# artiom-matvei/RLAO

Hardware: AMD Instinct MI355X
Metric: AO env-steps/sec (batched loops) (higher is better)
Workload: dtype f32; 1 GPU; 8m / 20x20 Shack-Hartmann, 256 batched envs per GPU, integrator closed loop (BASELINE.json configs[1]); envs_per_gpu=256, envs_total=256, resolution=120, n_valid_act=357, n_signal=632, layers=1, controller=leaky integrator, gain 0.5, noise=photon, parallelism=env-shards x1, all-gather of episode returns

## Files before the change

rlao_amd/csrc/common.hpp:

```cpp
#pragma once
#include <hip/hip_runtime.h>
#include <stdint.h>
#include <stddef.h>

#include <string>
#include <vector>

#include "aoenv.h"

namespace ao {

constexpr int kWave = 64;
constexpr int kMaxLayer = 8;
constexpr int kMtN = 624;
constexpr int kMaxSplits = 16;
constexpr int kMaxModes = 512;

int fail(const char* fmt, ...);
#define AO_HIP(call)                                                                          \
    do {                                                                                      \
        hipError_t e_ = (call);                                                               \
        if (e_ != hipSuccess)                                                                 \
            return ::ao::fail("%s:%d: %s -> %s", __FILE__, __LINE__, #call, hipGetErrorString(e_)); \
    } while (0)
// ... 29 lines not shown
    w[1] = 0.5 * (3 * x * x * x - 5 * x * x + 2);
    w[2] = 0.5 * (-3 * x * x * x + 4 * x * x + x);
    w[3] = 0.5 * (x * x * x - x * x);
}

__host__ __device__ inline bool clock_subpixel(const double ratio[2], double buff[2], int* bx, int* by) {
#pragma clang fp contract(off)
    for (int d = 0; d < 2; ++d) buff[d] += fmod(fabs(ratio[d]), 1.0) * clock_sgn(ratio[d]);
    *bx = fabs(buff[0]) < 1 ? 0 : (int)clock_sgn(buff[0]);
    *by = fabs(buff[1]) < 1 ? 0 : (int)clock_sgn(buff[1]);
    for (int d = 0; d < 2; ++d) buff[d] = fmod(fabs(buff[d]), 1.0) * clock_sgn(buff[d]);
    return *bx != 0 || *by != 0;
}

__host__ __device__ inline void taps_from_buff(const double buff[2], LayerTaps& t) {
#pragma clang fp contract(off)
    const double fy = -buff[1], fx = -buff[0];
    const double ky = floor(fy), kx = floor(fx);
    t.dy = (int)ky;
    t.dx = (int)kx;
    catmull_rom(fy - ky, t.wy);
    catmull_rom(fx - kx, t.wx);
}

struct PhaseArgs {
    const void* screen[kMaxLayer];
    const void* minmax[kMaxLayer];
    LayerTaps taps[kMaxLayer];
    int n_layer;
    int S;
    int foot;
    int S_l[kMaxLayer];
    int foot_l[kMaxLayer];
    int update_atm;
    int store_atm;
    int store_phase;
    int minmax_dirty[kMaxLayer];
    const LayerTaps* env_taps;
    int n_env;
};

__device__ inline const LayerTaps& layer_taps(const PhaseArgs& pa, int l, int e) {
    return pa.env_taps ? pa.env_taps[(size_t)l * pa.n_env + e] : pa.taps[l];
}

}

namespace ao {

struct Env;

template <typename T>
int launch_ring_prepare(const T* map, T* zx, const int* inner_idx, const uint32_t* mt_state, const int* mt_pos,
                        uint32_t* mt_state_out, int* mt_pos_out, const int* env_idx, int n, int S, int n_inner, int n_outer, int K,
                        int sx, int sy, int oy, int ox, const double* xi_scale, hipStream_t st);
template <typename T>
int launch_mt_normal(uint32_t* mt_state, int* mt_pos, T* zx, int n_env, int K, int n_inner, int n_outer,
                     const double* xi_scale, hipStream_t st);
template <typename T>
int launch_scatter_minmax(T* new_map, const T* X, const int* outer_idx, T* minmax, const int* env_idx, int n, int n_env, int S,
                          int n_outer, int splits, int oy, int ox, int with_minmax, hipStream_t st, const LayerTaps* env_taps = nullptr);
template <typename T>
int launch_ring_prepare_env(const T* map, T* zx, const int* inner_idx, uint32_t* mt_state, int* mt_pos, const EnvClock* clk_in,
                            EnvClock* clk_out, LayerTaps* taps, double weight, int n_env, int S, int n_inner, int n_outer, int K,
                            const double* xi_scale, hipStream_t st);
template <typename T>
int launch_minmax(const T* maps, T* minmax, int n_env, int S, hipStream_t st);
int launch_mt_seed(const uint32_t* seeds, int stride, const int* env_idx, uint32_t* mt_state, int* mt_pos, int n, hipStream_t st);
template <typename T>
int launch_reset_env_rows(const int* env_idx, int n_idx, T* coefs, T* dm_prev, int n_valid_act, EnvClock* clk, LayerTaps* taps,
                          int n_layer, int n_env, hipStream_t st);
int gemm_splits(int M, int N, int K);
struct MtAhead {
    const uint32_t* mt_in;
    const int* pos_in;
    uint32_t* mt_out;
    int* pos_out;
    float* zx_out;
    int K, n_inner, n_outer, n_env;
    const double* xi_scale;
};
int launch_ring_gemm_draw_ahead(const float* X, const float* W, float* Cpart, int M, int N, int K, int splits, const MtAhead& m,
                                hipStream_t st);
int launch_sum_slabs(float* x, size_t n, int slabs, hipStream_t st);
int launch_gemm_nt_mfma(const float* X, const float* W, float* Cpart, int M, int N, int K, int ldx, int ldw, int splits,
                        hipStream_t st, int xsplits = 1, size_t xslab = 0);
template <typename T>
int launch_gemm_nt(const T* X, const T* W, T* C, int M, int N, int K, int ldx, int ldw, int ldc, hipStream_t st);

__host__ __device__ inline size_t ga_index(int x, int k, int ga_stride) {
    const int q = k & 3, s = k >> 2;
    return ((((size_t)(x >> 4) * (ga_stride >> 2) + (s >> 2)) * 4 + q) * 16 + (x & 15)) * 4 + (s & 3);
}
template <typename T>
struct PhaseBuffers {
    T* opd_atm;
    const T* coefs;
    const T* coefs_img;
    const T* dm_opd;
    const T* gx;
    const T* gy;
    const T* gxt;
    const float* gxa;
    const float* gya;
    int ga_stride;
    const float* s1a;
    const int* act_idx;
    const uint8_t* pupil;
    T* phase;
    double* part;
    T* wfs_max;
};
int phase_tiles(int R, int n_act, size_t esz);
template <typename T>
int launch_coefs_image(const T* coefs, const int* act_idx, T* img, int n_env, int n_act, int n_valid_act, hipStream_t st);
int launch_dm_rows(const float* coefs, const int* act_idx, const float* gya, float* s1a, int n_env, int R, int n_act, int n_valid_act,
                   int ga_stride, hipStream_t st);
template <typename T>
struct KArgs {
    PhaseArgs pa;
    PhaseBuffers<T> pb;
    int R, n_act, n_valid_act, tx, rp;
    T atm_scale;
    T src_scale;
};
template <typename T>
KArgs<T> make_phase_kargs(const PhaseArgs& pa, const PhaseBuffers<T>& pb, int R, int n_act, int n_valid_act,
                          double atm_wavelength, double src_wavelength);
template <typename T>
int launch_phase(const PhaseArgs& pa, const PhaseBuffers<T>& pb, int n_env, int R, int n_act, int n_valid_act,
                 double atm_wavelength, double src_wavelength, bool use_mfma, int force_path, hipStream_t st);

template <typename T>
struct ShConst {
    const T* amp;
    const int* subap_idx;
    const uint8_t* valid2d;
    const T* ref;
    const T* tw;
    const T* ph;
    T units;
    T threshold;
    int fast_trig;
};
template <typename T>
int launch_sh_spots(const T* phase, const ShConst<T>& sc, T* frame, T* wfs_max, int n_env, int R, int n_subap,
                    int n_valid, hipStream_t st);
template <typename T>
int launch_sh_centroid(const T* frame, const T* wfs_max, const ShConst<T>& sc, T* signal, int n_env, int R,
                       int n_subap, int n_valid, int max_group, hipStream_t st);

template <typename T>
struct FinishArgs {
    const T* v;
    int splits;
    const int* act_idx;
    const T* action;
    T* coefs;
    T* dm_prev;
    T* obs;
    T* reward;
    T* ret;
    T* strehl;
    T* scal;
    T* total;
    T* residual;
// ... 120 lines not shown
```

rlao_amd/csrc/env.hip:

```cpp
#include <algorithm>
#include <cmath>
#include <cstdarg>
#include <cstdio>
#include <cstring>
#include <initializer_list>
#include <new>
#include <utility>

#include "common.hpp"
#include "detector.hpp"
#include "sh_device.hpp"

namespace ao {

static thread_local std::string g_err;

int fail(const char* fmt, ...) {
    char buf[1024];
    va_list ap;
    va_start(ap, fmt);
    vsnprintf(buf, sizeof(buf), fmt, ap);
    va_end(ap);
    g_err = buf;
    return 1;
// ... 202 lines not shown
    sc.fast_trig = (env->use_fast_trig && sizeof(T) == 4) ? 1 : 0;
    return sc;
}

template <typename T>
int gemm_dispatch(AoEnv* env, const T* X, const T* W, T* C, int M, int N, int K, int* splits, hipStream_t st);
template <>
int gemm_dispatch<float>(AoEnv* env, const float* X, const float* W, float* C, int M, int N, int K, int* splits,
                         hipStream_t st) {
    if (!env->use_mfma) { *splits = 1; return launch_gemm_nt<float>(X, W, C, M, N, K, K, K, N, st); }
    *splits = gemm_splits(M, N, K);
    return launch_gemm_nt_mfma(X, W, C, M, N, K, K, K, *splits, st);
}
template <>
int gemm_dispatch<double>(AoEnv*, const double* X, const double* W, double* C, int M, int N, int K, int* splits,
                          hipStream_t st) {
    *splits = 1;
    return launch_gemm_nt<double>(X, W, C, M, N, K, K, K, N, st);
}

void forget_lookahead(Layer& y) { y.ahead.valid = false; y.gather_next = false; }

void drop_ring(Layer& y) { y.ring_pending = 0; }

void move_origin(Layer& y, int sx, int sy) {
    y.org[0] = ((y.org[0] - sy) % y.S + y.S) % y.S;
    y.org[1] = ((y.org[1] - sx) % y.S + y.S) % y.S;
}

void defer_ring(AoEnv* env, int l, const void* zx, int splits) {
    env->last_zx = zx;
    env->last_zx_layer = l;
    env->layer[l].ring_pending = splits;
    env->layer[l].ring_src = env->xbuf_ptr(l);
}

void take_rings(AoEnv* env, StepArgs& a) {
    for (int l = 0; l < env->L; ++l) {
        Layer& y = env->layer[l];
        a.ring_x[l] = y.ring_pending ? static_cast<const float*>(y.ring_src) : nullptr;
        a.ring_splits[l] = y.ring_pending;
        const bool g = y.gather_next && y.ring_pending && y.ahead.valid;
        a.next_zx[l] = g ? static_cast<float*>(env->zx_pipe_ptr(y.ahead.buf, l)) : nullptr;
        a.next_sx[l] = y.ahead.sx;
        a.next_sy[l] = y.ahead.sy;
        if (y.gather_next && !g) y.ahead.valid = false;
        y.gather_next = false;
    }
}

void rings_written(AoEnv* env) {
    for (int l = 0; l < env->L; ++l) { env->layer[l].ring_pending = 0; env->layer[l].minmax_dirty = false; }
}

template <typename T>
int scatter_ring(AoEnv* env, int l, const LayerTaps* et, bool with_minmax, hipStream_t st) {
    Layer& y = env->layer[l];
    AO_PROF(env, SCATTER, st);
    AO_TRY(launch_scatter_minmax<T>(env->as<T>(env->screen_ptr(l)), static_cast<const T*>(y.ring_src), y.outer_idx,
                                    env->as<T>(env->minmax_ptr(l)), nullptr, env->E, env->E, y.S, y.nout, y.ring_pending, y.org[0],
                                    y.org[1], with_minmax ? 1 : 0, st, et));
    y.ring_pending = 0;
    return 0;
}

template <typename T>
int flush_ring(AoEnv* env, int l, hipStream_t st) {
    Layer& y = env->layer[l];
    if (!y.ring_pending) return 0;
    if (y.gather_next) forget_lookahead(y);
    const LayerTaps* et = env->per_env_wind ? env->env_taps + (size_t)l * env->E : nullptr;
    return scatter_ring<T>(env, l, et, et != nullptr, st);
}
template <typename T>
int flush_rings(AoEnv* env, hipStream_t st) {
    for (int l = 0; l < env->L; ++l) AO_TRY(flush_ring<T>(env, l, st));
    return 0;
}

template <typename T>
int ring_gemm(AoEnv* env, int l, const T* zx, int* splits, hipStream_t st) {
    const Layer& y = env->layer[l];
    AO_PROF(env, GEMM_RING, st);
    return gemm_dispatch<T>(env, zx, env->as<T>(y.ab), env->as<T>(env->xbuf_ptr(l)), env->E, y.nout, y.K, splits, st);
}

template <typename T>
int extrude(AoEnv* env, int l, int sx, int sy, bool lean, hipStream_t st, bool defer = false) {
    Layer& y = env->layer[l];
    forget_lookahead(y);
    AO_TRY(flush_ring<T>(env, l, st));
    T* zx = env->as<T>(env->zx);
    {
        AO_PROF(env, SHIFT_GATHER, st);
        AO_TRY(launch_ring_prepare<T>(env->as<T>(env->screen_ptr(l)), zx, y.inner_idx, y.mt_cur, y.pos_cur, y.mt_cur, y.pos_cur, nullptr,
                                      env->E, y.S, y.nin, y.nout, y.K, sx, sy, y.org[0], y.org[1], env->sigma(), st));
    }
    int splits = 1;
    AO_TRY(ring_gemm<T>(env, l, zx, &splits, st));
    move_origin(y, sx, sy);
    defer_ring(env, l, zx, splits);
    if (!(defer && lean)) AO_TRY(scatter_ring<T>(env, l, nullptr, !lean, st));
    y.minmax_dirty = lean;
    return 0;
}

template <typename T>
int first_ring(AoEnv* env, int l, const int* d_idx, int n, hipStream_t st) {
    Layer& y = env->layer[l];
    T* zx = env->as<T>(env->zx);
    T* map = env->as<T>(env->screen_ptr(l));
    {
        AO_PROF(env, SHIFT_GATHER, st);
        AO_TRY(launch_ring_prepare<T>(map, zx, y.inner_idx, y.mt_cur, y.pos_cur, y.mt_cur, y.pos_cur, d_idx, n, y.S, y.nin, y.nout, y.K, 0, 0,
                                      0, 0, env->sigma(), st));
    }
    int splits = 1;
    AO_TRY(ring_gemm<T>(env, l, zx, &splits, st));
    env->last_zx = zx;
    env->last_zx_layer = l;
    {
        AO_PROF(env, SCATTER, st);
        AO_TRY(launch_scatter_minmax<T>(map, env->as<T>(env->xbuf_ptr(l)), y.outer_idx, env->as<T>(env->minmax_ptr(l)), d_idx, n, env->E,
                                        y.S, y.nout, splits, 0, 0, 1, st));
    }
    if (!d_idx) y.minmax_dirty = false;
    return 0;
}

template <typename T>
int refresh_minmax(AoEnv* env, hipStream_t st) {
    AO_TRY(flush_rings<T>(env, st));
    for (int l = 0; l < env->L; ++l)
        if (env->layer[l].minmax_dirty) {
            AO_TRY(launch_minmax<T>(env->as<T>(env->screen_ptr(l)), env->as<T>(env->minmax_ptr(l)), env->E, env->layer[l].S, st));
            env->layer[l].minmax_dirty = false;
        }
    return 0;
}

bool next_crossing(const LayerClock& k0, int* sx, int* sy) {
    if ((int)std::fabs(k0.ratio[0]) > 0 || (int)std::fabs(k0.ratio[1]) > 0) return false;
    if (k0.ratio[0] == 0 && k0.ratio[1] == 0) return false;
    double b[2] = {k0.buff[0], k0.buff[1]};
    for (int it = 0; it < 1000000; ++it) {
        for (int d = 0; d < 2; ++d) b[d] += std::fmod(std::fabs(k0.ratio[d]), 1.0) * sgn(k0.ratio[d]);
        if (std::fabs(b[0]) >= 1 || std::fabs(b[1]) >= 1) {
            *sx = std::fabs(b[0]) < 1 ? 0 : (int)sgn(b[0]);
            *sy = std::fabs(b[1]) < 1 ? 0 : (int)sgn(b[1]);
            return true;
        }
        for (int d = 0; d < 2; ++d) b[d] = std::fmod(std::fabs(b[d]), 1.0) * sgn(b[d]);
    }
    return false;
}

int extrude_pipelined(AoEnv* env, int l, int sx, int sy, hipStream_t st) {
    Layer& y = env->layer[l];
    const int cur = y.ahead.buf;
    float* op = static_cast<float*>(env->zx_pipe_ptr(cur, l));
    if (y.ahead.valid && y.ahead.sx == sx && y.ahead.sy == sy) {
        std::swap(y.mt_cur, y.mt_alt);
        std::swap(y.pos_cur, y.pos_alt);
    } else {
        AO_PROF(env, SHIFT_GATHER, st);
        AO_TRY(launch_ring_prepare<float>(env->as<float>(env->screen_ptr(l)), op, y.inner_idx, y.mt_cur, y.pos_cur, y.mt_cur, y.pos_cur,
                                          nullptr, env->E, y.S, y.nin, y.nout, y.K, sx, sy, y.org[0], y.org[1], env->sigma(), st));
    }
    forget_lookahead(y);
    const int splits = gemm_splits(env->E, y.nout, y.K);
    MtAhead m{y.mt_cur, y.pos_cur, y.mt_alt, y.pos_alt, static_cast<float*>(env->zx_pipe_ptr(1 - cur, l)), y.K, y.nin, y.nout, env->E,
              env->sigma()};
    {
        AO_PROF(env, GEMM_RING, st);
        AO_TRY(launch_ring_gemm_draw_ahead(op, env->as<float>(y.ab), static_cast<float*>(env->xbuf_ptr(l)), env->E, y.nout, y.K, splits, m,
                                           st));
    }
    move_origin(y, sx, sy);
    defer_ring(env, l, op, splits);
    y.minmax_dirty = true;
    int nsx = 0, nsy = 0;
    if (next_crossing(y.clk, &nsx, &nsy)) {
        y.ahead = RingAhead{true, nsx, nsy, 1 - cur};
        y.gather_next = true;
    }
    return 0;
}

template <typename T>
int advance_atmosphere_env(AoEnv* env, bool lean, hipStream_t st) {
    for (int l = 0; l < env->L; ++l) {
        AO_TRY(flush_ring<T>(env, l, st));
        const Layer& y = env->layer[l];
        T* zx = env->as<T>(env->zx);
        const size_t row = (size_t)l * env->E;
        {
            AO_PROF(env, SHIFT_GATHER, st);
            AO_TRY(launch_ring_prepare_env<T>(env->as<T>(env->screen_ptr(l)), zx, y.inner_idx, y.mt_cur, y.pos_cur,
                                              env->env_clk[env->clk_cur] + row, env->env_clk[1 - env->clk_cur] + row, env->env_taps + row,
                                              y.weight, env->E, y.S, y.nin, y.nout, y.K, env->sigma(), st));
        }
        int splits = 1;
        AO_TRY(ring_gemm<T>(env, l, zx, &splits, st));
        defer_ring(env, l, zx, splits);
        if (!(lean && env->defer_ring)) AO_TRY(flush_ring<T>(env, l, st));
    }
    env->clk_cur = 1 - env->clk_cur;
    return 0;
}

template <typename T>
int advance_atmosphere(AoEnv* env, bool lean, hipStream_t st) {
    if (env->per_env_wind) return advance_atmosphere_env<T>(env, lean, st);
    for (int l = 0; l < env->L; ++l) {
        LayerClock& k = env->layer[l].clk;
        if (k.ratio[0] == 0 && k.ratio[1] == 0) continue;
        const int ns[2] = {(int)std::fabs(k.ratio[0]), (int)std::fabs(k.ratio[1])};
        const int mn = ns[0] < ns[1] ? ns[0] : ns[1], mx = ns[0] > ns[1] ? ns[0] : ns[1];
        const int s0 = (int)sgn(k.ratio[0]), s1 = (int)sgn(k.ratio[1]);
        for (int i = 0; i < mn; ++i) AO_TRY(extrude<T>(env, l, s0, s1, lean, st));
        for (int j = 0; j < mx - mn; ++j)
            AO_TRY(extrude<T>(env, l, ns[0] == mn ? 0 : s0, ns[1] == mn ? 0 : s1, lean, st));
        int b0, b1;
        if (clock_subpixel(k.ratio, k.buff, &b0, &b1)) {
            if (lean && env->defer_ring && env->use_lookahead && env->zx_pipe && !env->layer[l].ring_pending) {
                AO_TRY(extrude_pipelined(env, l, b0, b1, st));
            } else {
                AO_TRY(extrude<T>(env, l, b0, b1, lean, st, lean && env->defer_ring));
            }
        }
    }
    return 0;
}

template <typename T>
void fill_phase_args(AoEnv* env, PhaseArgs& pa, PhaseBuffers<T>& pb, int update_atm, int store_atm, int store_phase);

template <typename T>
int run_phase(AoEnv* env, int update_atm, int store_atm, hipStream_t st, int store_phase = 1) {
    AO_TRY(refresh_minmax<T>(env, st));
    if (env->use_coefs_img && env->c.dm_separable) {
        if constexpr (std::is_same<T, float>::value) {
            if (env->dm_rows)
                AO_TRY(launch_dm_rows(env->as<float>(env->coefs), env->act_idx, env->gya, env->dm_rows, env->E, env->R, env->nAct, env->A,
                                      env->ga_stride, st));
        }
        if (env->coefs_img)
            AO_TRY(launch_coefs_image<T>(env->as<T>(env->coefs), env->act_idx, env->as<T>(env->coefs_img), env->E, env->nAct, env->A, st));
    }
    PhaseArgs pa;
    PhaseBuffers<T> pb;
    fill_phase_args<T>(env, pa, pb, update_atm, store_atm, store_phase);
    AO_PROF(env, PHASE, st);
    return launch_phase<T>(pa, pb, env->E, env->R, env->nAct, env->A, env->c.atm_wavelength, env->c.src_wavelength,
                           env->use_mfma, env->force_path, st);
}

template <typename T>
int apply_detector(AoEnv* env, bool sh, hipStream_t st) {
    if (!env->det.active) return 0;
    env->det.frame_counter += 1;
    AO_PROF(env, DETECTOR, st);
// ... 1551 lines not shown
```

rlao_amd/csrc/gemm_kernels.hip:

```cpp
#include "common.hpp"
#include "ring_device.hpp"

namespace ao {

template <typename T>
__global__ void __launch_bounds__(256) k_gemm_nt(const T* __restrict__ X, const T* __restrict__ W, T* __restrict__ C,
                                                 int M, int N, int K, int ldx, int ldw, int ldc) {
    constexpr int BM = 64, BN = 64, BK = 16;
    __shared__ T xs[BK][BM + 1];
    __shared__ T ws[BK][BN + 1];
    const int m0 = blockIdx.y * BM, n0 = blockIdx.x * BN;
    const int tx = threadIdx.x % 16, ty = threadIdx.x / 16;
    T acc[4][4];
#pragma unroll
    for (int i = 0; i < 4; ++i)
#pragma unroll
        for (int j = 0; j < 4; ++j) acc[i][j] = (T)0;

    for (int k0 = 0; k0 < K; k0 += BK) {
        for (int q = threadIdx.x; q < BM * BK; q += 256) {
            const int r = q / BK, kk = q % BK;
            const int gm = m0 + r, gn = n0 + r, gk = k0 + kk;
            xs[kk][r] = (gm < M && gk < K) ? X[(size_t)gm * ldx + gk] : (T)0;
            ws[kk][r] = (gn < N && gk < K) ? W[(size_t)gn * ldw + gk] : (T)0;
// ... 63 lines not shown
                if (gm < M) {
                    xv[pass] = *reinterpret_cast<const float4*>(X + (size_t)gm * ldx + gk);
                    for (int z = 1; z < xsplits; ++z) {
                        const float4 t = *reinterpret_cast<const float4*>(X + (size_t)z * xslab + (size_t)gm * ldx + gk);
                        xv[pass].x += t.x; xv[pass].y += t.y; xv[pass].z += t.z; xv[pass].w += t.w;
                    }
                }
                if (gn < N) wv[pass] = *reinterpret_cast<const float4*>(W + (size_t)gn * ldw + gk);
            } else {
                float* xp = reinterpret_cast<float*>(&xv[pass]);
                float* wp = reinterpret_cast<float*>(&wv[pass]);
                for (int d = 0; d < 4; ++d) {
                    if (gk + d < kend) {
                        if (gm < M) {
                            xp[d] = X[(size_t)gm * ldx + gk + d];
                            for (int z = 1; z < xsplits; ++z) xp[d] += X[(size_t)z * xslab + (size_t)gm * ldx + gk + d];
                        }
                        if (gn < N) wp[d] = W[(size_t)gn * ldw + gk + d];
                    }
                }
            }
        }
    };
    if (kbeg < kend) fetch(kbeg);
    for (int k0 = kbeg; k0 < kend; k0 += BK) {
#pragma unroll
        for (int pass = 0; pass < 2; ++pass) {
            const int r = (threadIdx.x >> 3) + pass * 32, kq = (threadIdx.x & 7) * 4;
            float* xd = xs + r * LDT + kq;
            float* wd = ws + r * LDT + kq;
            xd[0] = xv[pass].x; xd[1] = xv[pass].y; xd[2] = xv[pass].z; xd[3] = xv[pass].w;
            wd[0] = wv[pass].x; wd[1] = wv[pass].y; wd[2] = wv[pass].z; wd[3] = wv[pass].w;
        }
        __syncthreads();
        if (k0 + BK < kend) fetch(k0 + BK);
        const float* xa = xs + (wm + lr) * LDT + lh;
        const float* wb = ws + (wn + lr) * LDT + lh;
#pragma unroll
        for (int kk = 0; kk < BK / 2; ++kk)
            acc = __builtin_amdgcn_mfma_f32_32x32x2f32(xa[2 * kk], wb[2 * kk], acc, 0, 0, 0);
        __syncthreads();
    }
    float* C = Cpart + (size_t)bz * M * N;
    const int gn = n0 + wn + lr;
    if (gn < N) {
#pragma unroll
        for (int rg = 0; rg < 16; ++rg) {
            const int gm = m0 + wm + (rg & 3) + 8 * (rg >> 2) + 4 * lh;
            if (gm < M) C[(size_t)gm * N + gn] = acc[rg];
        }
    }
}

__global__ void __launch_bounds__(256) k_gemm_nt_mfma(const float* __restrict__ X, const float* __restrict__ W,
                                                      float* __restrict__ Cpart, int M, int N, int K, int ldx,
                                                      int ldw, int kslice, int xsplits, size_t xslab) {
    gemm_nt_mfma_tile(X, W, Cpart, M, N, K, ldx, ldw, kslice, xsplits, xslab, (int)blockIdx.z);
}

__global__ void __launch_bounds__(256) k_ring_gemm_draw_ahead(const float* __restrict__ X, const float* __restrict__ W,
                                                              float* __restrict__ Cpart, int M, int N, int K, int ldx, int ldw,
                                                              int kslice, int splits, const MtAhead m) {
    const int draw_slices = (int)gridDim.z - splits;
    if ((int)blockIdx.z >= draw_slices) {
        gemm_nt_mfma_tile(X, W, Cpart, M, N, K, ldx, ldw, kslice, 1, 0, (int)blockIdx.z - draw_slices);
        return;
    }
    const int e = ((int)blockIdx.z * (int)gridDim.y + (int)blockIdx.y) * (int)gridDim.x + (int)blockIdx.x;
    if (e < m.n_env) mt_normal_body<float>(m.mt_in, m.pos_in, m.mt_out, m.pos_out, m.zx_out, m.K, m.n_inner, m.n_outer, e,
                                           m.xi_scale);
}

int launch_ring_gemm_draw_ahead(const float* X, const float* W, float* Cpart, int M, int N, int K, int splits, const MtAhead& m,
                                hipStream_t st) {
    if (m.n_outer % 2) return fail("mt_normal: n_outer=%d must be even", m.n_outer);
    const int kslice = cdiv(cdiv(K, splits), 32) * 32;
    const int gx = cdiv(N, 64), gy = cdiv(M, 64);
    dim3 grid(gx, gy, splits + cdiv(m.n_env, gx * gy));
    hipLaunchKernelGGL(k_ring_gemm_draw_ahead, grid, dim3(256), 0, st, X, W, Cpart, M, N, K, K, K, kslice, splits, m);
    AO_HIP(hipGetLastError());
    return 0;
}

int gemm_splits(int M, int N, int K) {
    const int tiles = cdiv(M, 64) * cdiv(N, 64);
    if (K > 2048) {
        int best = 1;
        double best_cost = 1e300;
        for (int s = 1; s <= kMaxSplits; ++s) {
            const int wgs = tiles * s, kslice = cdiv(cdiv(K, s), 32) * 32;
            if (wgs < 1024 && s < kMaxSplits && tiles * (s + 1) <= 1024) continue;
            const double cost = (double)cdiv(wgs, 256) * (kslice + 96) + (double)s * M * N * 8.0 / 4e12 / 20e-9;
            if (cost < best_cost) { best_cost = cost; best = s; }
        }
        return best;
    }
    (void)tiles;
    const int smax = K / 64 > 0 ? K / 64 : 1;
    return smax > kMaxSplits ? kMaxSplits : smax;
}

__global__ void __launch_bounds__(256) k_sum_slabs(float* __restrict__ x, int n4, int slabs, size_t slab4) {
    const int i = blockIdx.x * 256 + threadIdx.x;
    if (i >= n4) return;
    float4* p = reinterpret_cast<float4*>(x);
    float4 v[kMaxSplits];
#pragma unroll
    for (int z = 0; z < kMaxSplits; ++z) v[z] = p[(size_t)(z < slabs ? z : 0) * slab4 + i];
    float4 a = v[0];
#pragma unroll
    for (int z = 1; z < kMaxSplits; ++z)
        if (z < slabs) { a.x += v[z].x; a.y += v[z].y; a.z += v[z].z; a.w += v[z].w; }
    p[i] = a;
}
int launch_sum_slabs(float* x, size_t n, int slabs, hipStream_t st) {
    if (n % 4) return fail("sum_slabs: %zu elements per slab, not a multiple of 4", n);
    hipLaunchKernelGGL(k_sum_slabs, dim3(cdiv((int)(n / 4), 256)), dim3(256), 0, st, x, (int)(n / 4), slabs, n / 4);
    AO_HIP(hipGetLastError());
    return 0;
}

int launch_gemm_nt_mfma(const float* X, const float* W, float* Cpart, int M, int N, int K, int ldx, int ldw, int splits,
                        hipStream_t st, int xsplits, size_t xslab) {
    const int kslice = cdiv(cdiv(K, splits), 32) * 32;
    dim3 grid(cdiv(N, 64), cdiv(M, 64), splits);
    hipLaunchKernelGGL(k_gemm_nt_mfma, grid, dim3(256), 0, st, X, W, Cpart, M, N, K, ldx, ldw, kslice, xsplits, xslab);
    AO_HIP(hipGetLastError());
    return 0;
}

template <typename T>
__global__ void __launch_bounds__(1024) k_recon_finish(const FinishArgs<T> f) {
    extern __shared__ __align__(16) unsigned char lds_raw[];
    T* img_s = reinterpret_cast<T*>(lds_raw);
    __shared__ double red[16];
    __shared__ double tel[4];
    const int e = blockIdx.x, n_env = gridDim.x;
    const int img = f.n_act * f.n_act;
    T* ob = f.obs + (size_t)e * img;
    const size_t slab = (size_t)n_env * f.n_valid_act;
    const T* vv = f.v + (size_t)e * f.n_valid_act;
    for (int q = threadIdx.x; q < img; q += blockDim.x) img_s[q] = (T)0;
    __syncthreads();
    double ss = 0.0;
    for (int k = threadIdx.x; k < f.n_valid_act; k += blockDim.x) {
        const int px = f.act_idx[k];
        if (f.do_integrate) {
            const T a = (f.gain_from_obs != (T)0) ? f.gain_from_obs * ob[px] : f.action[(size_t)e * img + px];
            const size_t ck = (size_t)e * f.n_valid_act + k;
            const float af = (float)a;
            const T inc = ((T)af == a) ? (T)(af * 1e-6f) : a * (T)1e-6;
            const T cn = f.dm_prev[ck] * f.leak + inc;
            f.coefs[ck] = cn;
            f.dm_prev[ck] = cn;
        }
        T acc = vv[k];
        for (int z = 1; z < f.splits; ++z) acc += vv[(size_t)z * slab + k];
        const T o = -acc * (T)1e6;
        img_s[px] = o;
        ss += (double)o * (double)o;
    }
    double tv[4] = {0, 0, 0, 0};
    const bool tel_wave = threadIdx.x / kWave == blockDim.x / kWave - 1;
    if (tel_wave) {
        const double* pp = f.part + (size_t)e * f.n_tiles * 4;
        for (int t = threadIdx.x & (kWave - 1); t < f.n_tiles; t += kWave)
// ... 70 lines not shown
```

rlao_amd/csrc/ring_device.hpp:

```cpp
#pragma once
#include "common.hpp"

namespace ao {

__device__ inline int torus(int r, int c, int oy, int ox, int S) {
    int pr = r + oy, pc = c + ox;
    pr = pr >= S ? pr - S : pr;
    pc = pc >= S ? pc - S : pc;
    return pr * S + pc;
}

template <typename T>
__device__ inline void gather_ring(const T* __restrict__ map, T* __restrict__ zx, const int* __restrict__ inner_idx, int S,
                                   int n_inner, int K, int sx, int sy, int oy, int ox, int e, int t0, int nt) {
    const T* src = map + (size_t)e * S * S;
    for (int k = t0; k < n_inner; k += nt) {
        const int idx = inner_idx[k];
        const int r = idx / S - sy, c = idx % S - sx;
        zx[(size_t)e * K + k] = src[torus(r, c, oy, ox, S)];
    }
}

__device__ inline uint32_t mt_temper(uint32_t y) {
    y ^= (y >> 11);
    y ^= (y << 7) & 0x9d2c5680u;
    y ^= (y << 15) & 0xefc60000u;
    y ^= (y >> 18);
    return y;
}

__device__ inline uint32_t mt_mix(uint32_t a, uint32_t b, uint32_t far) {
    uint32_t y = (a & 0x80000000u) | (b & 0x7fffffffu);
    return far ^ (y >> 1) ^ ((y & 1u) ? 0x9908b0dfu : 0u);
}

__device__ inline void mt_twist(uint32_t* s) {
    const int t = threadIdx.x;
    uint32_t v = 0;
    if (t < 227) v = mt_mix(s[t], s[t + 1], s[t + 397]);
    __syncthreads();
    if (t < 227) s[t] = v;
    __syncthreads();
    if (t < 227) v = mt_mix(s[t + 227], s[t + 228], s[t]);
    __syncthreads();
    if (t < 227) s[t + 227] = v;
    __syncthreads();
    if (t < 169) v = mt_mix(s[t + 454], s[t + 455], s[t + 227]);
    __syncthreads();
    if (t < 169) s[t + 454] = v;
    __syncthreads();
    if (t == 0) s[623] = mt_mix(s[623], s[0], s[396]);
    __syncthreads();
}

template <typename T>
__device__ inline void mt_normal_body(const uint32_t* mt_state, const int* mt_pos, uint32_t* mt_state_out, int* mt_pos_out,
                                      T* __restrict__ zx, int K, int n_inner, int n_outer, int e, const double* xi_scale) {
    __shared__ uint32_t s[kMtN];
    __shared__ int scan[256];
    __shared__ int sh_pos, sh_got, sh_stop;
    const int t = threadIdx.x;
    const uint32_t* gs = mt_state + (size_t)e * kMtN;
    uint32_t* gso = mt_state_out + (size_t)e * kMtN;
    for (int i = t; i < kMtN; i += 256) s[i] = gs[i];
    if (t == 0) {
        sh_pos = mt_pos[e];
        sh_got = 0;
    }
    __syncthreads();
    const int need_pairs = n_outer / 2;
    T* out = zx + (size_t)e * K + n_inner;
    while (true) {
        if (sh_pos >= kMtN) {
            mt_twist(s);
            if (t == 0) sh_pos = 0;
            __syncthreads();
        }
        const int pos = sh_pos, got = sh_got;
        const int avail = (kMtN - pos) / 4;
        int acc = 0;
        double n0 = 0.0, n1 = 0.0;
        if (t < avail) {
            const uint32_t* w = s + pos + 4 * t;
            const double d1 = ((double)(mt_temper(w[0]) >> 5) * 67108864.0 + (double)(mt_temper(w[1]) >> 6)) /
                              9007199254740992.0;
            const double d2 = ((double)(mt_temper(w[2]) >> 5) * 67108864.0 + (double)(mt_temper(w[3]) >> 6)) /
                              9007199254740992.0;
            const double x1 = 2.0 * d1 - 1.0, x2 = 2.0 * d2 - 1.0;
            const double r2 = x1 * x1 + x2 * x2;
            if (r2 < 1.0 && r2 != 0.0) {
                acc = 1;
                const double f = sqrt(-2.0 * log(r2) / r2);
                n0 = f * x2;
                n1 = f * x1;
                if (xi_scale) {
                    const double sg = xi_scale[e];
                    n0 *= sg;
                    n1 *= sg;
                }
            }
        }
        const unsigned long long bal = __ballot(acc);
        const int lane = t & (kWave - 1), wv = t / kWave;
        const int in_wave = __popcll(bal & ((lane == 63) ? ~0ull : ((2ull << lane) - 1ull)));
        if (lane == 0) scan[wv] = __popcll(bal);
        __syncthreads();
        int before = 0;
        for (int q = 0; q < wv; ++q) before += scan[q];
        const int total_acc = scan[0] + scan[1] + scan[2] + scan[3];
        const int incl = before + in_wave;
        const int remaining = need_pairs - got;
        if (t == 0) sh_stop = -1;
        __syncthreads();
        if (acc && incl <= remaining) {
            const int j = got + incl - 1;
            out[2 * j] = (T)n0;
            out[2 * j + 1] = (T)n1;
            if (incl == remaining) sh_stop = t;
        }
        __syncthreads();
        if (sh_stop >= 0) {
            if (t == 0) sh_pos = pos + 4 * (sh_stop + 1);
            break;
        }
        if (t == 0) {
            sh_pos = kMtN;
            sh_got = got + total_acc;
        }
        __syncthreads();
    }
    __syncthreads();
    for (int i = t; i < kMtN; i += 256) gso[i] = s[i];
    if (t == 0) mt_pos_out[e] = sh_pos;
}

}
```

Before: 5.491 million env-steps/s.

## Fuse ring GEMM split-K reduction in-workgroup and batch MT draws per workgroup

Adds a single-launch ring product kernel. Each 1024-thread workgroup computes a 32x32 output tile with one wave per K slice using f32 MFMA and permlane swaps, then reduces the slices in LDS. This removes the separate slab-sum pass and the partial-sum buffers when K is small. The same launch hosts the Mersenne-Twister normal draws for the next step, with four envs per workgroup. Those draws are restructured to twist three state blocks ahead and try two candidates per lane, which cuts the number of barriered passes. The risks are register pressure from 1024-thread blocks and more complex RNG bookkeeping that must keep sequences identical.

```diff
diff --git a/rlao_amd/csrc/common.hpp b/rlao_amd/csrc/common.hpp
--- a/rlao_amd/csrc/common.hpp
+++ b/rlao_amd/csrc/common.hpp
@@ -135,6 +135,8 @@
 };
 int launch_ring_gemm_draw_ahead(const float* X, const float* W, float* Cpart, int M, int N, int K, int splits, const MtAhead& m,
                                 hipStream_t st);
+inline bool ring_one_slab(int K) { return K <= 2048; }
+int launch_ring_product(const float* X, const float* W, float* C, int M, int N, int K, int splits, const MtAhead* m, hipStream_t st);
 int launch_sum_slabs(float* x, size_t n, int slabs, hipStream_t st);
 int launch_gemm_nt_mfma(const float* X, const float* W, float* Cpart, int M, int N, int K, int ldx, int ldw, int splits,
                         hipStream_t st, int xsplits = 1, size_t xslab = 0);
diff --git a/rlao_amd/csrc/env.hip b/rlao_amd/csrc/env.hip
--- a/rlao_amd/csrc/env.hip
+++ b/rlao_amd/csrc/env.hip
@@ -308,6 +308,13 @@
 int ring_gemm(AoEnv* env, int l, const T* zx, int* splits, hipStream_t st) {
     const Layer& y = env->layer[l];
     AO_PROF(env, GEMM_RING, st);
+    if constexpr (std::is_same<T, float>::value) {
+        if (env->use_mfma && ring_one_slab(y.K)) {
+            *splits = 1;
+            return launch_ring_product(zx, env->as<float>(y.ab), env->as<float>(env->xbuf_ptr(l)), env->E, y.nout, y.K,
+                                       gemm_splits(env->E, y.nout, y.K), nullptr, st);
+        }
+    }
     return gemm_dispatch<T>(env, zx, env->as<T>(y.ab), env->as<T>(env->xbuf_ptr(l)), env->E, y.nout, y.K, splits, st);
 }
 
@@ -397,13 +404,15 @@
     const int splits = gemm_splits(env->E, y.nout, y.K);
     MtAhead m{y.mt_cur, y.pos_cur, y.mt_alt, y.pos_alt, static_cast<float*>(env->zx_pipe_ptr(1 - cur, l)), y.K, y.nin, y.nout, env->E,
               env->sigma()};
+    const bool one_slab = ring_one_slab(y.K);
     {
         AO_PROF(env, GEMM_RING, st);
-        AO_TRY(launch_ring_gemm_draw_ahead(op, env->as<float>(y.ab), static_cast<float*>(env->xbuf_ptr(l)), env->E, y.nout, y.K, splits, m,
-                                           st));
+        float* x = static_cast<float*>(env->xbuf_ptr(l));
+        if (one_slab) AO_TRY(launch_ring_product(op, env->as<float>(y.ab), x, env->E, y.nout, y.K, splits, &m, st));
+        else AO_TRY(launch_ring_gemm_draw_ahead(op, env->as<float>(y.ab), x, env->E, y.nout, y.K, splits, m, st));
     }
     move_origin(y, sx, sy);
-    defer_ring(env, l, op, splits);
+    defer_ring(env, l, op, one_slab ? 1 : splits);
     y.minmax_dirty = true;
     int nsx = 0, nsy = 0;
     if (next_crossing(y.clk, &nsx, &nsy)) {
diff --git a/rlao_amd/csrc/gemm_kernels.hip b/rlao_amd/csrc/gemm_kernels.hip
--- a/rlao_amd/csrc/gemm_kernels.hip
+++ b/rlao_amd/csrc/gemm_kernels.hip
@@ -169,6 +169,112 @@
     return 0;
 }
 
+constexpr int kRingBufs = 3;
+constexpr int kRingLds = kMaxSplits * 32 * 32 * (int)sizeof(float);
+static_assert(4 * sizeof(MtLds) <= (size_t)kRingLds, "the four streams of a draw workgroup fit the product's LDS");
+
+__device__ inline float4 ring_load4(const float* __restrict__ row, int gk, int kend, bool vec_ok) {
+    if (vec_ok && gk + 3 < kend) return *reinterpret_cast<const float4*>(row + gk);
+    float4 v;
+    v.x = gk < kend ? row[gk] : 0.f;
+    v.y = gk + 1 < kend ? row[gk + 1] : 0.f;
+    v.z = gk + 2 < kend ? row[gk + 2] : 0.f;
+    v.w = gk + 3 < kend ? row[gk + 3] : 0.f;
+    return v;
+}
+
+__device__ inline void half_swap(float& a, float& b) {
+    const auto r = __builtin_amdgcn_permlane32_swap(__float_as_uint(a), __float_as_uint(b), false, false);
+    a = __uint_as_float(r[0]);
+    b = __uint_as_float(r[1]);
+}
+
+__device__ inline void ring_product_tile(const float* __restrict__ X, const float* __restrict__ W, float* __restrict__ C, int M, int N,
+                                         int K, int kslice, int splits, int tile, float* red) {
+    const int tiles_n = (N + 31) / 32;
+    const int m0 = (tile / tiles_n) * 32, n0 = (tile % tiles_n) * 32;
+    const int z = threadIdx.x / kWave, lane = threadIdx.x & (kWave - 1);
+    const int lr = lane & 31, lh = lane >> 5;
+    if (z < splits) {
+        const int kbeg = z * kslice, kend = min(K, kbeg + kslice);
+        const int rounds = kbeg < kend ? (kend - kbeg + 31) / 32 : 0;
+        const float* xr = X + (size_t)min(m0 + lr, M - 1) * K;
+        const float* wr = W + (size_t)min(n0 + lr, N - 1) * K;
+        const bool vec_ok = (K & 3) == 0;
+        f32x16 acc;
+#pragma unroll
+        for (int i = 0; i < 16; ++i) acc[i] = 0.f;
+        for (int c0 = 0; c0 < rounds; c0 += kRingBufs) {
+            float4 xv[kRingBufs][4], wv[kRingBufs][4];
+#pragma unroll
+            for (int b = 0; b < kRingBufs; ++b)
+                if (c0 + b < rounds) {
+#pragma unroll
+                    for (int j = 0; j < 4; ++j) {
+                        const int gk = kbeg + (c0 + b) * 32 + 8 * j + 4 * lh;
+                        xv[b][j] = ring_load4(xr, gk, kend, vec_ok);
+                        wv[b][j] = ring_load4(wr, gk, kend, vec_ok);
+                    }
+                }
+#pragma unroll
+            for (int b = 0; b < kRingBufs; ++b)
+                if (c0 + b < rounds) {
+#pragma unroll
+                    for (int j = 0; j < 4; ++j) {
+                        float4 x = xv[b][j], w = wv[b][j];
+                        half_swap(x.x, x.y);
+                        half_swap(x.z, x.w);
+                        half_swap(w.x, w.y);
+                        half_swap(w.z, w.w);
+                        acc = __builtin_amdgcn_mfma_f32_32x32x2f32(x.x, w.x, acc, 0, 0, 0);
+                        acc = __builtin_amdgcn_mfma_f32_32x32x2f32(x.z, w.z, acc, 0, 0, 0);
+                        acc = __builtin_amdgcn_mfma_f32_32x32x2f32(x.y, w.y, acc, 0, 0, 0);
+                        acc = __builtin_amdgcn_mfma_f32_32x32x2f32(x.w, w.w, acc, 0, 0, 0);
+                    }
+                }
+        }
+        float* rz = red + z * 1024 + lr;
+#pragma unroll
+        for (int rg = 0; rg < 16; ++rg) rz[((rg & 3) + 8 * (rg >> 2) + 4 * lh) * 32] = acc[rg];
+    }
+    __syncthreads();
+    const int t = threadIdx.x;
+    float sv[kMaxSplits];
+#pragma unroll
+    for (int q = 0; q < kMaxSplits; ++q) sv[q] = red[(q < splits ? q : 0) * 1024 + t];
+    float v = sv[0];
+#pragma unroll
+    for (int q = 1; q < kMaxSplits; ++q)
+        if (q < splits) v += sv[q];
+    const int gm = m0 + (t >> 5), gn = n0 + (t & 31);
+    if (gm < M && gn < N) C[(size_t)gm * N + gn] = v;
+}
+
+__global__ void __launch_bounds__(1024) k_ring_product(const float* __restrict__ X, const float* __restrict__ W, float* __restrict__ C,
+                                                       int M, int N, int K, int kslice, int splits, int draw_wgs, const MtAhead m) {
+    __shared__ __align__(16) unsigned char lds[kRingLds];
+    if ((int)blockIdx.x < draw_wgs) {
+        MtLds* ml = reinterpret_cast<MtLds*>(lds);
+        const int g = threadIdx.x / kMtLanes, e = (int)blockIdx.x * 4 + g;
+        mt_normal_streams<float>(ml, 4, ml[g], threadIdx.x % kMtLanes, e < m.n_env, m.mt_in, m.pos_in, m.mt_out, m.pos_out, m.zx_out,
+                                 m.K, m.n_inner, m.n_outer, e, m.xi_scale);
+        return;
+    }
+    ring_product_tile(X, W, C, M, N, K, kslice, splits, (int)blockIdx.x - draw_wgs, reinterpret_cast<float*>(lds));
+}
+
+int launch_ring_product(const float* X, const float* W, float* C, int M, int N, int K, int splits, const MtAhead* m, hipStream_t st) {
+    if (splits < 1 || splits > kMaxSplits) return fail("ring product: %d slices", splits);
+    if (m && m->n_outer % 2) return fail("mt_normal: n_outer=%d must be even", m->n_outer);
+    const int kslice = cdiv(cdiv(K, splits), 32) * 32;
+    const int draw_wgs = m ? cdiv(m->n_env, 4) : 0;
+    const MtAhead none{};
+    hipLaunchKernelGGL(k_ring_product, dim3(draw_wgs + cdiv(M, 32) * cdiv(N, 32)), dim3(1024), 0, st, X, W, C, M, N, K, kslice, splits,
+                       draw_wgs, m ? *m : none);
+    AO_HIP(hipGetLastError());
+    return 0;
+}
+
 int gemm_splits(int M, int N, int K) {
     const int tiles = cdiv(M, 64) * cdiv(N, 64);
     if (K > 2048) {
diff --git a/rlao_amd/csrc/ring_device.hpp b/rlao_amd/csrc/ring_device.hpp
--- a/rlao_amd/csrc/ring_device.hpp
+++ b/rlao_amd/csrc/ring_device.hpp
@@ -34,104 +34,139 @@
     return far ^ (y >> 1) ^ ((y & 1u) ? 0x9908b0dfu : 0u);
 }
 
-__device__ inline void mt_twist(uint32_t* s) {
-    const int t = threadIdx.x;
-    uint32_t v = 0;
-    if (t < 227) v = mt_mix(s[t], s[t + 1], s[t + 397]);
+__device__ inline void mt_twist(const uint32_t* a, uint32_t* b, int t, bool on) {
+    if (on && t < 227) b[t] = mt_mix(a[t], a[t + 1], a[t + 397]);
     __syncthreads();
-    if (t < 227) s[t] = v;
+    if (on && t < 227) b[t + 227] = mt_mix(a[t + 227], a[t + 228], b[t]);
     __syncthreads();
-    if (t < 227) v = mt_mix(s[t + 227], s[t + 228], s[t]);
+    if (on && t < 169) b[t + 454] = mt_mix(a[t + 454], a[t + 455], b[t + 227]);
+    if (on && t == 0) b[623] = mt_mix(a[623], b[0], b[396]);
     __syncthreads();
-    if (t < 227) s[t + 227] = v;
+}
+
+__device__ inline bool mt_polar(const uint32_t* w, double* n0, double* n1) {
+    const double d1 = ((double)(mt_temper(w[0]) >> 5) * 67108864.0 + (double)(mt_temper(w[1]) >> 6)) / 9007199254740992.0;
+    const double d2 = ((double)(mt_temper(w[2]) >> 5) * 67108864.0 + (double)(mt_temper(w[3]) >> 6)) / 9007199254740992.0;
+    const double x1 = 2.0 * d1 - 1.0, x2 = 2.0 * d2 - 1.0;
+    const double r2 = x1 * x1 + x2 * x2;
+    if (!(r2 < 1.0 && r2 != 0.0)) return false;
+    const double f = sqrt(-2.0 * log(r2) / r2);
+    *n0 = f * x2;
+    *n1 = f * x1;
+    return true;
+}
+
+constexpr int kMtLanes = 256;
+constexpr int kMtBlocks = 3;
+constexpr int kMtBlockTries = kMtN / 4;
+static_assert(kMtBlockTries * kMtBlocks <= 2 * kMtLanes, "two attempts per lane cover one pass");
+
+struct MtLds {
+    uint32_t s[kMtBlocks][kMtN];
+    int scan[2][kMtLanes / kWave];
+    int pos, got, stop, done;
+};
+
+template <typename T>
+__device__ inline void mt_normal_streams(MtLds* lds, int n_streams, MtLds& L, int t, bool live, const uint32_t* mt_state,
+                                         const int* mt_pos, uint32_t* mt_state_out, int* mt_pos_out, T* __restrict__ zx, int K,
+                                         int n_inner, int n_outer, int e, const double* xi_scale) {
+    const uint32_t* gs = mt_state + (size_t)e * kMtN;
+    uint32_t* gso = mt_state_out + (size_t)e * kMtN;
+    if (live)
+        for (int i = t; i < kMtN; i += kMtLanes) L.s[0][i] = gs[i];
+    if (t == 0) {
+        L.pos = live ? mt_pos[e] : kMtN;
+        L.got = 0;
+        L.stop = -1;
+        L.done = live ? 0 : 1;
+    }
     __syncthreads();
-    if (t < 169) v = mt_mix(s[t + 454], s[t + 455], s[t + 227]);
-    __syncthreads();
-    if (t < 169) s[t + 454] = v;
-    __syncthreads();
-    if (t == 0) s[623] = mt_mix(s[623], s[0], s[396]);
-    __syncthreads();
+    const int need_pairs = n_outer / 2;
+    T* out = zx + (size_t)e * K + n_inner;
+    const int lane = t & (kWave - 1), wv = t / kWave;
+    const unsigned long long upto = (lane == 63) ? ~0ull : ((2ull << lane) - 1ull);
+    while (true) {
+        const bool on = !L.done;
+        mt_twist(L.s[0], L.s[1], t, on);
+        mt_twist(L.s[1], L.s[2], t, on);
+        const int pos = L.pos, got = L.got;
+        const int avail0 = (kMtN - pos) / 4;
+        const int avail = avail0 + (kMtBlocks - 1) * kMtBlockTries;
+        int acc[2] = {0, 0};
+        double n0[2] = {0.0, 0.0}, n1[2] = {0.0, 0.0};
+#pragma unroll
+        for (int r = 0; r < 2; ++r) {
+            const int i = t + r * kMtLanes;
+            if (on && i < avail) {
+                const int j = i - avail0;
+                const uint32_t* w = j < 0 ? L.s[0] + pos + 4 * i : L.s[1 + j / kMtBlockTries] + 4 * (j % kMtBlockTries);
+                if (mt_polar(w, &n0[r], &n1[r])) {
+                    acc[r] = 1;
+                    if (xi_scale) {
+                        const double sg = xi_scale[e];
+                        n0[r] *= sg;
+                        n1[r] *= sg;
+                    }
+                }
+            }
+        }
+        const unsigned long long bal0 = __ballot(acc[0]), bal1 = __ballot(acc[1]);
+        if (lane == 0) {
+            L.scan[0][wv] = __popcll(bal0);
+            L.scan[1][wv] = __popcll(bal1);
+        }
+        __syncthreads();
+        int total0 = 0, total1 = 0, before0 = 0, before1 = 0;
+#pragma unroll
+        for (int q = 0; q < kMtLanes / kWave; ++q) {
+            const int c0 = L.scan[0][q], c1 = L.scan[1][q];
+            total0 += c0;
+            total1 += c1;
+            if (q < wv) { before0 += c0; before1 += c1; }
+        }
+        const int incl[2] = {before0 + (int)__popcll(bal0 & upto), total0 + before1 + (int)__popcll(bal1 & upto)};
+        const int remaining = need_pairs - got;
+#pragma unroll
+        for (int r = 0; r < 2; ++r)
+            if (acc[r] && incl[r] <= remaining) {
+                const int j = got + incl[r] - 1;
+                out[2 * j] = (T)n0[r];
+                out[2 * j + 1] = (T)n1[r];
+                if (incl[r] == remaining) L.stop = t + r * kMtLanes;
+            }
+        __syncthreads();
+        if (on) {
+            const int stop = L.stop;
+            if (stop >= 0) {
+                const int j = stop - avail0;
+                const int blk = j < 0 ? 0 : 1 + j / kMtBlockTries;
+                for (int i = t; i < kMtN; i += kMtLanes) gso[i] = L.s[blk][i];
+                if (t == 0) {
+                    mt_pos_out[e] = j < 0 ? pos + 4 * (stop + 1) : 4 * (j % kMtBlockTries + 1);
+                    L.done = 1;
+                }
+            } else {
+                for (int i = t; i < kMtN; i += kMtLanes) L.s[0][i] = L.s[kMtBlocks - 1][i];
+                if (t == 0) {
+                    L.pos = kMtN;
+                    L.got = got + total0 + total1;
+                }
+            }
+        }
+        __syncthreads();
+        bool more = false;
+        for (int g = 0; g < n_streams; ++g) more = more || !lds[g].done;
+        if (!more) break;
+    }
 }
 
 template <typename T>
 __device__ inline void mt_normal_body(const uint32_t* mt_state, const int* mt_pos, uint32_t* mt_state_out, int* mt_pos_out,
                                       T* __restrict__ zx, int K, int n_inner, int n_outer, int e, const double* xi_scale) {
-    __shared__ uint32_t s[kMtN];
-    __shared__ int scan[256];
-    __shared__ int sh_pos, sh_got, sh_stop;
-    const int t = threadIdx.x;
-    const uint32_t* gs = mt_state + (size_t)e * kMtN;
-    uint32_t* gso = mt_state_out + (size_t)e * kMtN;
-    for (int i = t; i < kMtN; i += 256) s[i] = gs[i];
-    if (t == 0) {
-        sh_pos = mt_pos[e];
-        sh_got = 0;
-    }
-    __syncthreads();
-    const int need_pairs = n_outer / 2;
-    T* out = zx + (size_t)e * K + n_inner;
-    while (true) {
-        if (sh_pos >= kMtN) {
-            mt_twist(s);
-            if (t == 0) sh_pos = 0;
-            __syncthreads();
-        }
-        const int pos = sh_pos, got = sh_got;
-        const int avail = (kMtN - pos) / 4;
-        int acc = 0;
-        double n0 = 0.0, n1 = 0.0;
-        if (t < avail) {
-            const uint32_t* w = s + pos + 4 * t;
-            const double d1 = ((double)(mt_temper(w[0]) >> 5) * 67108864.0 + (double)(mt_temper(w[1]) >> 6)) /
-                              9007199254740992.0;
-            const double d2 = ((double)(mt_temper(w[2]) >> 5) * 67108864.0 + (double)(mt_temper(w[3]) >> 6)) /
-                              9007199254740992.0;
-            const double x1 = 2.0 * d1 - 1.0, x2 = 2.0 * d2 - 1.0;
-            const double r2 = x1 * x1 + x2 * x2;
-            if (r2 < 1.0 && r2 != 0.0) {
-                acc = 1;
-                const double f = sqrt(-2.0 * log(r2) / r2);
-                n0 = f * x2;
-                n1 = f * x1;
-                if (xi_scale) {
-                    const double sg = xi_scale[e];
-                    n0 *= sg;
-                    n1 *= sg;
-                }
-            }
-        }
-        const unsigned long long bal = __ballot(acc);
-        const int lane = t & (kWave - 1), wv = t / kWave;
-        const int in_wave = __popcll(bal & ((lane == 63) ? ~0ull : ((2ull << lane) - 1ull)));
-        if (lane == 0) scan[wv] = __popcll(bal);
-        __syncthreads();
-        int before = 0;
-        for (int q = 0; q < wv; ++q) before += scan[q];
-        const int total_acc = scan[0] + scan[1] + scan[2] + scan[3];
-        const int incl = before + in_wave;
-        const int remaining = need_pairs - got;
-        if (t == 0) sh_stop = -1;
-        __syncthreads();
-        if (acc && incl <= remaining) {
-            const int j = got + incl - 1;
-            out[2 * j] = (T)n0;
-            out[2 * j + 1] = (T)n1;
-            if (incl == remaining) sh_stop = t;
-        }
-        __syncthreads();
-        if (sh_stop >= 0) {
-            if (t == 0) sh_pos = pos + 4 * (sh_stop + 1);
-            break;
-        }
-        if (t == 0) {
-            sh_pos = kMtN;
-            sh_got = got + total_acc;
-        }
-        __syncthreads();
-    }
-    __syncthreads();
-    for (int i = t; i < kMtN; i += 256) gso[i] = s[i];
-    if (t == 0) mt_pos_out[e] = sh_pos;
+    __shared__ MtLds lds;
+    mt_normal_streams<T>(&lds, 1, lds, threadIdx.x, true, mt_state, mt_pos, mt_state_out, mt_pos_out, zx, K, n_inner, n_outer, e,
+                         xi_scale);
 }
 
 }
```

After: 5.150 million env-steps/s. 6.2% lower.
